# jessegrabowski/gEconpy

Measured on AMD Instinct MI355X. Metric: solve+Kalman-logp evals/sec, Smets-Wouters n~40 T=200, higher is better.
Workload: dtype f64; 1 GPU; sw_shaped synthetic (SURVEY 8d): n=m=40, n_state=18, n_lead=12, k=7, p=7, T_len=200, 4096 draws per GPU (BASELINE configs[2]); global_batch=4096, solver=cycle_reduction, inputs=A,B,C,D resident in HBM, parallelism=single GPU

## Files before the change

geconpy_amd/_lib.py:

```python
from __future__ import annotations

import ctypes as C
import os

PKG = os.path.dirname(os.path.abspath(__file__))
LIB_PATH = os.path.join(PKG, "libdsge_hip.so")

ABI_VERSION = 19
ERR_INVALID, ERR_HIP, ERR_TOO_LARGE = 1, 2, 3
MAX_N = 64
MAX_N_CR = 64
MAX_N_GENSYS = 64
MAX_N_BIG = 96
MAX_P = 16

ST_OK = 0
ST_NOT_CONVERGED = 1
ST_NAN = 2
ST_LYAP_FAIL = 4
ST_FILTER_NONFINITE = 8
ST_GENSYS_QZ_FAIL = 16
ST_GENSYS_TOO_BIG = 32
ST_GRAD_UNSUPPORTED = 64
ST_SECOND_ORDER_UNSUPPORTED = 128
# ... 39 lines not shown


class GensysForward(C.Structure):

    _fields_ = [("f_mat", C.c_void_p), ("f_wt", C.c_void_p), ("y_wt", C.c_void_p), ("loose", C.c_void_p),
                ("n_unstable", C.c_void_p), ("pi_raw", C.c_int32)]


_INTS = ("N T_len batch bound_batched c c_batched correlation cv_batched cv_paths d_batched device enable eps_batched "
         "eta_batched full_cov h_batched horizon k lag_step m max_iter mode n n_cond n_eta n_filter_hint n_grid n_groups n_lags "
         "n_lead n_lead_hint n_links n_out n_paths n_ret n_shock_steps n_state n_state_hint n_steps nnz p q_batched q_mode "
         "remainder reps s_batched shock solver w_batched x0_batched x0_paths z_batched z_selector_hint")
_KINDS = {**dict.fromkeys(_INTS.split(), C.c_int), **dict.fromkeys("jitter missing_fill rank_tol tol".split(), C.c_double),
          "scratch_limit_bytes": C.c_size_t}
_OBS = "Z z_batched d d_batched Hdiag h_batched"
_FILTER = f"T R Q q_mode {_OBS} y batch m k p T_len jitter missing_fill"
_FUSED = f"A B C D Q q_mode {_OBS} y batch n k p T_len solver tol max_iter jitter missing_fill"
_LOGP = f"{_FUSED} n_state_hint z_selector_hint n_lead_hint logp_out status_out"
_GRAD = f"A B C D q q_batched {_OBS} y batch n k p T_len solver tol max_iter jitter missing_fill"
_BARS = "logp_out status_out A_bar B_bar C_bar D_bar q_bar d_bar h_bar"
_PRUNED = "T R gyy gyu guu gss state_idx n_state"
_PENCIL = "g0 g1 *c psi pi batch N k n_eta tol G1_out C_out impact_out gev_out eu_out status"
_DEVICE_ENTRIES = {
    "dsge_abi_version": "",
    "dsge_last_error": "",
    "dsge_device_count": "",
    "dsge_set_device": "device",
    "dsge_stream_synchronize": "stream",
    "dsge_options_init": "opt",
    "dsge_options_push": "opt",
    "dsge_options_pop": "",
    "dsge_forget_measured_shapes": "",
    "dsge_debug_cr_phases": "enable cycles_out",
    "dsge_debug_kalman_steady_steps": "steady_at_device",
    "dsge_debug_kalman_timeline": "timeline_device",
    "dsge_debug_kalman_phases": "enable cycles_out",
    "dsge_debug_big_phases": "enable cycles_out",
    "dsge_debug_gensys_phases": "A B C batch n tol n_lead_hint T_out eu_out status cycles_out",
    "dsge_debug_gensys_window_phases": "enable cycles_out",
    "dsge_debug_gensys_stage_ms": "enable ms_out",
    "dsge_debug_adjoint_refine": "mode",
    "dsge_debug_second_order_phases": "enable cycles_out",
    "dsge_debug_pruned_phases": "enable cycles_out",
    "dsge_debug_shock_decomp_phases": "enable cycles_out",
    "dsge_debug_condfc_phases": "enable cycles_out",
    "dsge_profile_pipeline": f"{_LOGP} reps ms_out stream",
    "dsge_cycle_reduction_batched": "A B C batch n max_iter tol T_out status n_iter stream",
    "dsge_scan_cycle_reduction_batched": "A B C batch n max_iter tol T_out status *n_steps stream",
    "dsge_gensys_batched": "A B C D batch n k tol n_lead_hint T_out R_out eu_out status stream",
    "dsge_gensys_pencil_batched": f"{_PENCIL} stream",
    "dsge_gensys_pencil_full_batched": f"{_PENCIL} forward stream",
    "dsge_bk_eigenvalues_batched": "A B C batch n tol eig_re eig_im n_eig n_forward n_unstable status stream",
    "dsge_selection_batched": "A B C D T batch n k R_out resid_out stream",
    "dsge_policy_adjoints_batched": "B C T T_bar batch n A_bar B_bar C_bar status stream",
    "dsge_selection_adjoints_batched": "B C T R R_bar batch n k B_bar C_bar D_bar T_bar stream",
    "dsge_policy_norms_batched": "A B C D T R state_mask batch n k det_norm_out stoch_norm_out stream",
    "dsge_backward_direct_batched": "A B D batch n k T_out R_out stream",
    "dsge_lyapunov_batched": "T R Q q_mode batch m k P0_out RQR_out status stream",
    "dsge_autocorrelation_batched": "T R Q q_mode Z Hdiag batch m k p n_lags lag_step correlation acf_out Sigma_out status stream",
    "dsge_kalman_logp_batched": f"{_FILTER} n_state_hint z_selector_hint logp_out status_io stream",
    "dsge_kalman_filter_outputs_batched": f"{_FILTER} ll_out a_pred_out a_filt_out p_pred_out p_filt_out full_cov status_io stream",
    "dsge_kalman_smoother_batched": (f"{_FILTER} rank_tol scratch_limit_bytes ll_out a_smooth_out p_smooth_out eps_smooth_out "
                                     "full_cov status_io stream"),
    "dsge_simulation_smoother_batched": (f"{_FILTER} rank_tol scratch_limit_bytes x0 x0_batched eps eps_batched eta eta_batched "
                                         "n_paths ll_out x_out eps_out status_io stream"),
    "dsge_simulate_batched": "T R eps eps_batched x0 x0_batched status batch m k n_paths n_steps n_shock_steps x_out stream",
# ... 188 lines not shown
```

geconpy_amd/csrc/dsge_api.hip:

```cpp
#include <hip/hip_runtime.h>

#include <cmath>
#include <cstdio>
#include <cstdlib>
#include <cstring>
#include <mutex>
#include <string>
#include <vector>

#include "dsge_host.hpp"

namespace {
thread_local std::string g_last_error;
}

namespace dsge_host {
int fail(int code, const std::string& msg) {
  g_last_error = msg;
  return code;
}
static Options defaults_from_environment() {
  Options o;
  if (const char* e = std::getenv("DSGE_GENSYS_DOUBLING"))
    if ((e[0] >= '0' && e[0] <= '3') && e[1] == '\0') o.gensys_doubling = e[0] - '0';
// ... 224 lines not shown

namespace {
thread_local ThreadStream t_verdict;
constexpr int MAX_CHUNK_STREAMS = 8;
thread_local ThreadStream t_chunk[MAX_CHUNK_STREAMS];

StreamArenaPool g_scratch_pool;
StreamArenaPool g_aug_big_pool;
}

extern "C" {

int dsge_abi_version(void) { return DSGE_ABI_VERSION; }
const char* dsge_last_error(void) { return g_last_error.c_str(); }

static int debug_counters(long long** slot, int count, int enable, long long* cycles_out) {
  int rc = ensure_device();
  if (rc) return rc;
  if (enable && !*slot) {
    HIP_TRY(hipMalloc((void**)slot, count * sizeof(long long)));
    HIP_TRY(hipMemset(*slot, 0, count * sizeof(long long)));
  }
  if (cycles_out && *slot) {
    HIP_TRY(hipDeviceSynchronize());
    HIP_TRY(hipMemcpy(cycles_out, *slot, count * sizeof(long long), hipMemcpyDeviceToHost));
  }
  if (!enable && *slot) {
    (void)hipFree(*slot);
    *slot = nullptr;
  }
  return DSGE_SUCCESS;
}
int dsge_debug_cr_phases(int enable, long long* cycles_out) { return debug_counters(&g_cr_dbg, 8, enable, cycles_out); }
int dsge_debug_second_order_phases(int enable, long long* cycles_out) { return debug_counters(&g_so_dbg, 8, enable, cycles_out); }
int dsge_debug_pruned_phases(int enable, long long* cycles_out) { return debug_counters(&g_pruned_dbg, 8, enable, cycles_out); }
int dsge_debug_shock_decomp_phases(int enable, long long* cycles_out) { return debug_counters(&g_shock_decomp_dbg, 8, enable, cycles_out); }
int dsge_debug_condfc_phases(int enable, long long* cycles_out) { return debug_counters(&g_condfc_dbg, 8, enable, cycles_out); }
int dsge_debug_adjoint_refine(int mode) {
  if (mode < 0 || mode > 2) return fail(DSGE_ERR_INVALID, "mode out of range (0..2)");
  g_adj_refine_mode = mode;
  return DSGE_SUCCESS;
}
int dsge_forget_measured_shapes(void) {
  cr_deflation_reset();
  gensys_shape_reset();
  return DSGE_SUCCESS;
}
int dsge_debug_kalman_steady_steps(int32_t* steady_at_device) {
  g_kalman_steady_at = steady_at_device;
  return DSGE_SUCCESS;
}
int dsge_debug_kalman_timeline(long long* timeline_device) {
  g_kalman_timeline = timeline_device;
  return DSGE_SUCCESS;
}

int dsge_device_count(void) {
  int count = 0;
  if (hipGetDeviceCount(&count) != hipSuccess) {
    (void)hipGetLastError();
    return 0;
  }
  int ok = 0;
  for (int i = 0; i < count; ++i) {
    hipDeviceProp_t prop;
    if (hipGetDeviceProperties(&prop, i) == hipSuccess && std::strncmp(prop.gcnArchName, "gfx950", 6) == 0) ++ok;
// ... 1318 lines not shown
```

geconpy_amd/csrc/dsge_cr_compact.hpp:

```cpp
#pragma once
#include "dsge_device.hpp"

#include "../../include/dsge_hip.h"

namespace dsge {

template <int BS>
struct CrcSmem {
  static constexpr int NP = Tile<BS>::NP, LDW = 2 * NP + (BS % 2 == 0 ? 2 : 1);
  static constexpr size_t bytes = sizeof(double) * (size_t)(NP * LDW + NP * BS + BS * 2 * NP) + sizeof(int) * 5 * NP;
};

template <int BS>
__device__ __forceinline__ unsigned long long blk_colmask(const double (&x)[BS][BS]) {
  unsigned long long mask = 0ull;
#pragma unroll
  for (int j = 0; j < BS; ++j) {
    bool nz = false;
#pragma unroll
    for (int i = 0; i < BS; ++i) nz = nz || (x[i][j] != 0.0);
    unsigned long long b = __ballot(nz);
    b |= b >> 32;
    b |= b >> 16;
    b |= b >> 8;
    b &= 0xffull;
    while (b) {
      const int lcb = __ffsll((long long)b) - 1;
      b &= b - 1;
      const int col = lcb * BS + j;
      if (col < 64) mask |= 1ull << col;
    }
  }
  return mask;
}

template <int BS, typename IT>
__device__ __forceinline__ void crc_iterate(double (&A1)[BS][BS], double (&Ah)[BS][BS], double (&Rb)[BS][BS], double* W,
                                            double* Lbuf, double* Ybuf, int* prow, const IT* cmap, IT* rsrc,
                                            const IT* posS, const IT* posL, int n, int s, int l, int max_iter,
                                            double tol, int scan_mode, int lane_in, long long* ph, int& it, bool& converged,
                                            bool& saw_nan) {
  constexpr int NP = CrcSmem<BS>::NP, LDW = CrcSmem<BS>::LDW;
  double* G1 = W + NP;
// ... 65 lines not shown
    }
    wave_sync();
    if (ph) {
      const long long tk1 = clock64();
      ph[2] += tk1 - tk0;
      tk0 = tk1;
    }
    double acc1[BS][BS], acc2[BS][BS];
    blk_zero<BS>(acc1);
    blk_zero<BS>(acc2);
    mm_acc<BS, false>(acc1, G1, LDW, W, LDW, s, lr, lc);
    mm_acc<BS, false>(acc2, G1 + s, LDW, W + s * LDW, LDW, l, lr, lc);
    wave_sync();
    if (ph) {
      const long long tk1 = clock64();
      ph[3] += tk1 - tk0;
      tk0 = tk1;
    }
    blk_store_lds<BS>(acc1, W, LDW, lr, lc);
    blk_store_lds<BS>(acc2, G1, LDW, lr, lc);
    wave_sync();
    double t0[BS][BS], t2[BS][BS];
    int vS[BS], vL[BS];
#pragma unroll
    for (int j = 0; j < BS; ++j) {
      vS[j] = posS[lc * BS + j];
      vL[j] = posL[lc * BS + j];
    }
#pragma unroll
    for (int i = 0; i < BS; ++i)
#pragma unroll
      for (int j = 0; j < BS; ++j) {
        const int row = lr * BS + i, c = lc * BS + j;
        const double d02 = (vL[j] >= 0) ? W[row * LDW + vL[j]] : 0.0;
        const double d20 = (vS[j] >= 0) ? G1[row * LDW + vS[j]] : 0.0;
        A1[i][j] -= d02;
        A1[i][j] -= d20;
        Ah[i][j] -= d20;
        t0[i][j] = (c < s) ? acc1[i][j] : 0.0;
        t2[i][j] = (c >= s && c < wr) ? acc2[i][j] : 0.0;
        Rb[i][j] = -(t0[i][j] + t2[i][j]);
      }
    ++it;
    const double nrm0 = blk_norm1<BS>(t0);
    if (ph) ph[4] += clock64() - tk0;
    if (nrm0 < tol) {
      if (scan_mode || blk_norm1<BS>(t2) < tol) {
        converged = true;
        break;
      }
    } else if (nrm0 != nrm0) {
      saw_nan = true;
      break;
    }
    wave_sync();
  }
}

template <int BS>
__device__ __forceinline__ void cr_compact_body(const double* __restrict__ A, const double* __restrict__ B,
                                                const double* __restrict__ C, int batch, int n, int max_iter,
                                                double tol, double* __restrict__ T_out,
                                                int32_t* __restrict__ status,
                                                int32_t* __restrict__ n_iter_out,
                                                long long* __restrict__ dbg, int scan_mode,
                                                const double* __restrict__ D, int k,
                                                double* __restrict__ R_out) {
  constexpr int NP = CrcSmem<BS>::NP, LDW = CrcSmem<BS>::LDW;
// ... 1 lines not shown
  double* W = smem;
  double* G1 = W + NP;
  double* Lbuf = W + NP * LDW;
  double* Ybuf = Lbuf + NP * BS;
  int* prow = (int*)(Ybuf + BS * 2 * NP);
  int* cmap = prow + NP;
  int* posS = cmap + NP;
  int* posL = posS + NP;
  int* rsrc = posL + NP;
  const int lane = threadIdx.x, lr = lane >> 3, lc = lane & 7;

  for (int draw = blockIdx.x; draw < batch; draw = batch) {
    const size_t off = (size_t)draw * n * n;
    wave_sync();
    for (int idx = lane; idx < NP * LDW; idx += 64) W[idx] = 0.0;
    double A1[BS][BS], Ah[BS][BS], Rb[BS][BS];
    unsigned long long maskS, maskL;
    {
      double t[BS][BS];
      blk_load_global<BS>(t, A + off, n, n, n, lr, lc);
      maskS = blk_colmask<BS>(t);
      blk_load_global<BS>(t, C + off, n, n, n, lr, lc);
      maskL = blk_colmask<BS>(t);
    }
    const int s = __popcll(maskS), l = __popcll(maskL), wr = s + l;
    if (wr > NP) {
      if (lane == 0) status[draw] = DSGE_ST_INTERNAL_RERUN;
      continue;
    }
    if (lane < NP) {
      const unsigned long long below = (1ull << lane) - 1ull;
      const bool isS = (maskS >> lane) & 1ull, isL = (maskL >> lane) & 1ull;
      const int ps = __popcll(maskS & below), pl = s + __popcll(maskL & below);
      posS[lane] = isS ? ps : -1;
      posL[lane] = isL ? pl : -1;
      if (isS) cmap[ps] = lane;
      if (isL) cmap[pl] = lane;
    }
    wave_sync();
    int ccol[BS];
    int vS[BS], vL[BS];
#pragma unroll
    for (int j = 0; j < BS; ++j) {
      const int c = lc * BS + j;
      ccol[j] = (c < wr) ? cmap[c] : -1;
      vS[j] = posS[c];
      vL[j] = posL[c];
    }
#pragma unroll
    for (int i = 0; i < BS; ++i)
#pragma unroll
      for (int j = 0; j < BS; ++j) {
        const int r = lr * BS + i, c = lc * BS + j;
        double v = 0.0;
        if (r < n && ccol[j] >= 0) v = (c < s) ? A[off + (size_t)r * n + ccol[j]] : C[off + (size_t)r * n + ccol[j]];
        Rb[i][j] = v;
      }
    blk_load_global<BS>(A1, B + off, n, n, n, lr, lc);
#pragma unroll
    for (int i = 0; i < BS; ++i)
#pragma unroll
      for (int j = 0; j < BS; ++j) Ah[i][j] = A1[i][j];

    bool converged, saw_nan;
    int it;
    long long ph[8] = {0, 0, 0, 0, 0, 0, 0, 0};
    const long long tk_start = dbg ? clock64() : 0;
    crc_iterate<BS>(A1, Ah, Rb, W, Lbuf, Ybuf, prow, cmap, rsrc, posS, posL, n, s, l, max_iter, tol, scan_mode, lane,
// ... 2 lines not shown

    double Tb[BS][BS];
    blk_zero<BS>(Tb);
    const bool solve_T = converged || (scan_mode && !saw_nan);
    if (solve_T) {
      const bool want_R = (R_out != nullptr) && !scan_mode;
      const bool r_fits = want_R && (s + k <= NP);
      wave_sync();
      blk_store_lds<BS>(Ah, W, LDW, lr, lc);
      if (scan_mode && lr == lc) {
#pragma unroll
        for (int i = 0; i < BS; ++i) W[(lr * BS + i) * LDW + lc * BS + i] = Ah[i][i] + 1e-16;
      }
      {
        double t[BS][BS];
#pragma unroll
        for (int i = 0; i < BS; ++i)
#pragma unroll
          for (int j = 0; j < BS; ++j) {
            const int r = lr * BS + i, c = lc * BS + j;
            double v = 0.0;
            if (r < n && c < s) v = A[off + (size_t)r * n + ccol[j]];
            else if (r_fits && r < n && c >= s && c < s + k) v = D[(size_t)draw * n * k + (size_t)r * k + (c - s)];
            t[i][j] = v;
          }
        blk_store_lds<BS>(t, G1, LDW, lr, lc);
      }
      gauss_jordan_blocked<BS>(W, LDW, n, 2, Lbuf, Ybuf, prow, lane);
      gj_unpermute<BS>(W, LDW, n, 1, 2, prow, lane);
#pragma unroll
      for (int i = 0; i < BS; ++i)
#pragma unroll
        for (int j = 0; j < BS; ++j)
          Tb[i][j] = (vS[j] >= 0) ? -G1[(lr * BS + i) * LDW + vS[j]] : 0.0;
      if (r_fits) {
        for (int idx = lane; idx < n * k; idx += 64) {
          const int r = idx / k, c = idx - r * k;
          R_out[(size_t)draw * n * k + idx] = -G1[r * LDW + s + c];
        }
      } else if (want_R) {
        wave_sync();
        blk_store_lds<BS>(Ah, W, LDW, lr, lc);
        {
          double t[BS][BS];
          blk_load_global<BS>(t, D + (size_t)draw * n * k, n, k, k, lr, lc);
          blk_store_lds<BS>(t, G1, LDW, lr, lc);
        }
        gauss_jordan_blocked<BS>(W, LDW, n, 2, Lbuf, Ybuf, prow, lane);
        gj_unpermute<BS>(W, LDW, n, 1, 2, prow, lane);
        for (int idx = lane; idx < n * k; idx += 64) {
          const int r = idx / k, c = idx - r * k;
          R_out[(size_t)draw * n * k + idx] = -G1[r * LDW + c];
        }
      }
    }
    if (R_out != nullptr && !scan_mode && !solve_T)
      for (int idx = lane; idx < n * k; idx += 64) R_out[(size_t)draw * n * k + idx] = 0.0;
    blk_store_global<BS>(Tb, T_out + off, n, n, n, lr, lc);
    if (lane == 0) {
      status[draw] = solve_T ? DSGE_ST_OK : (DSGE_ST_NOT_CONVERGED | (saw_nan ? DSGE_ST_NAN : 0));
      if (n_iter_out) n_iter_out[draw] = it;
      if (dbg && draw == 0) {
        const long long tk_end = clock64();
        ph[5] = tk_end - tk_fin;
        ph[6] = tk_end - tk_start;
        ph[7] = it;
        for (int q = 0; q < 8; ++q) dbg[q] = ph[q];
// ... 27 lines not shown
```

geconpy_amd/csrc/dsge_cr_deflate.hpp:

```cpp
#pragma once
#include "dsge_device.hpp"

#include "../../include/dsge_hip.h"

namespace dsge {

constexpr int CRD_HMAX = 16;

__host__ __device__ inline size_t crd_top_doubles(int n, int k, int h) {
  return (size_t)h * (h + 3 * (n - h) + k) + 2;
}
__host__ __device__ inline size_t crd_deflate_smem(int tile) {
  return (size_t)(CRD_HMAX * tile + CRD_HMAX) * 8 + (64 + CRD_HMAX) * 4;
}
__host__ __device__ inline size_t crd_inflate_smem(int tile) {
  return (size_t)(2 * CRD_HMAX * tile + CRD_HMAX * CRD_HMAX + CRD_HMAX) * 8 + (64 + CRD_HMAX) * 4;
}

__global__ __launch_bounds__(64) void cr_static_scan_kernel(const double* __restrict__ A, const double* __restrict__ C,
                                                             int batch, int n, int32_t* __restrict__ out) {
  const int lane = threadIdx.x;
  for (int draw = blockIdx.x; draw < batch; draw += gridDim.x) {
    const size_t off = (size_t)draw * n * n;
    int nz = 0;
// ... 53 lines not shown
  }
  return keep;
}

template <typename IT>
__device__ __forceinline__ bool crd_col_source(int cv, const double* __restrict__ A, const double* __restrict__ B,
                                               const double* __restrict__ C, const double* __restrict__ D, size_t off,
                                               size_t offk, int n, int k, int h, const IT* dyi, const IT* sti,
                                               const double*& src, int& ss) {
  const int nd = n - h;
  src = B + off;
  ss = n;
  if (cv >= h + 3 * nd + k) return false;
  if (cv < h) {
    src = B + off + sti[cv];
    return true;
  }
  const int c = cv - h;
  if (c >= 3 * nd) {
    src = D + offk + (c - 3 * nd);
    ss = k;
    return true;
  }
  const int blk = (c >= nd) + (c >= 2 * nd);
  src = (blk == 0 ? B : (blk == 1 ? A : C)) + off + dyi[c - blk * nd];
  return true;
}

template <int NM, int NC, typename IT>
__device__ __forceinline__ void crd_qr_chunk(const double* __restrict__ A, const double* __restrict__ B,
                                             const double* __restrict__ C, const double* __restrict__ D, size_t off,
                                             size_t offk, int n, int k, int h, int c0, const IT* dyi, const IT* sti,
                                             double* V, double* __restrict__ tp, int lane, double (&col)[NC][NM],
                                             bool (&act)[NC], bool skip_zero_ac = false) {
  const int ncols = h + 3 * (n - h) + k;
  const double* src[NC];
  int ss[NC], cv[NC];
#pragma unroll
  for (int q = 0; q < NC; ++q) {
    cv[q] = c0 + 64 * q + lane;
    act[q] = crd_col_source(cv[q], A, B, C, D, off, offk, n, k, h, dyi, sti, src[q], ss[q]);
  }
#pragma unroll
  for (int r = 0; r < NM; ++r) {
    const int rr = r < n ? r : n - 1;
#pragma unroll
    for (int q = 0; q < NC; ++q) col[q][r] = src[q][(size_t)rr * ss[q]];
  }
  __builtin_amdgcn_sched_barrier(0);
#pragma unroll
  for (int r = 0; r < NM; ++r)
#pragma unroll
    for (int q = 0; q < NC; ++q) col[q][r] = (r < n && act[q]) ? col[q][r] : 0.0;
  bool wr[NC];
#pragma unroll
  for (int q = 0; q < NC; ++q) {
    wr[q] = act[q];
    if (skip_zero_ac) {
      bool nz = false;
#pragma unroll
      for (int r = 0; r < NM; ++r) nz = nz || (col[q][r] != 0.0);
      const int nd_ = n - h;
      const bool ac = cv[q] >= h + nd_ && cv[q] < h + 3 * nd_;
      wr[q] = act[q] && (nz || !ac);
    }
  }
  for (int j = 0; j < h; ++j) {
    double xn2 = 0.0, alpha;
    double d0[NC], d1[NC];
    if (c0 == 0) {
      if (lane == j) {
        double2* vw = reinterpret_cast<double2*>(V + j * NM);
#pragma unroll
        for (int r2 = 0; r2 < NM / 2; ++r2) vw[r2] = make_double2(col[0][2 * r2], col[0][2 * r2 + 1]);
      }
      wave_sync();
    }
    const double2* vj2 = reinterpret_cast<const double2*>(V + j * NM);
    {
      const double2 t0 = vj2[0];
      alpha = t0.x;
      xn2 = t0.y * t0.y;
#pragma unroll
      for (int q = 0; q < NC; ++q) {
        d0[q] = t0.y * col[q][1];
        d1[q] = 0.0;
      }
#pragma unroll
      for (int r2 = 1; r2 < NM / 2; ++r2) {
        const double2 t = vj2[r2];
        xn2 = fma(t.x, t.x, xn2);
#pragma unroll
        for (int q = 0; q < NC; ++q) d1[q] = fma(t.x, col[q][2 * r2], d1[q]);
        xn2 = fma(t.y, t.y, xn2);
#pragma unroll
        for (int q = 0; q < NC; ++q) d0[q] = fma(t.y, col[q][2 * r2 + 1], d0[q]);
      }
    }
    double beta = alpha, scal = 0.0, tj = 0.0;
    if (xn2 != 0.0) {
      const double nrm = sqrt(fma(alpha, alpha, xn2));
      beta = (alpha >= 0.0) ? -nrm : nrm;
      tj = (beta - alpha) / beta;
      scal = 1.0 / (alpha - beta);
    }
    const bool left = (c0 == 0) && (lane <= j);
    const double2 t0 = vj2[0];
#pragma unroll
    for (int q = 0; q < NC; ++q) {
      const bool lf = (q == 0) && left;
      const double w = lf ? 0.0 : -tj * fma(scal, d0[q] + d1[q], col[q][0]);
      const double topv = lf ? ((lane == j) ? beta : 0.0) : col[q][0] + w;
      if (wr[q]) tp[(size_t)j * ncols + cv[q]] = topv;
      const double ws = w * scal;
      col[q][0] = lf ? 0.0 : fma(t0.y, ws, col[q][1]);
#pragma unroll
      for (int r2 = 1; r2 < NM / 2; ++r2) {
        const double2 t = vj2[r2];
        col[q][2 * r2 - 1] = lf ? 0.0 : fma(t.x, ws, col[q][2 * r2]);
        col[q][2 * r2] = lf ? 0.0 : fma(t.y, ws, col[q][2 * r2 + 1]);
      }
      col[q][NM - 1] = 0.0;
    }
  }
}

template <int BS>
__global__ __launch_bounds__(64) void cr_deflate_kernel(const double* __restrict__ A, const double* __restrict__ B,
                                                         const double* __restrict__ C, const double* __restrict__ D,
                                                         int batch, int n, int k, int h, double* __restrict__ Ared,
                                                         double* __restrict__ Bred, double* __restrict__ Cred,
                                                         double* __restrict__ Dred, double* __restrict__ top,
                                                         int32_t* __restrict__ flag) {
  constexpr int NM = 8 * BS, HM = CRD_HMAX;
  extern __shared__ __attribute__((aligned(16))) double smem[];
  double* V = smem;
  double* tau_s = V + HM * NM;
  int* dyi = (int*)(tau_s + HM);
  int* sti = dyi + 64;
  const int lane = threadIdx.x;
  const int nd = n - h, nv = 3 * nd + k, ncols = h + nv;
  const size_t top_stride = crd_top_doubles(n, k, h);
  {
    const int draw = blockIdx.x;
    if (draw >= batch) return;
    const size_t off = (size_t)draw * n * n, offk = (size_t)draw * n * k;
    const size_t offr = (size_t)draw * nd * nd, offrk = (size_t)draw * nd * k;
    unsigned long long smask = crd_static_mask<NM>(A, C, off, n, lane);
    if (__popcll(smask) < h) {
      for (int idx = lane; idx < nd * nd; idx += 64) {
        Ared[offr + idx] = 0.0;
        Cred[offr + idx] = 0.0;
        Bred[offr + idx] = (idx / nd == idx % nd) ? 1.0 : 0.0;
// ... 240 lines not shown
```

geconpy_amd/csrc/dsge_cr_fused.hpp:

```cpp
#pragma once
#include "dsge_cr_compact.hpp"
#include "dsge_cr_deflate.hpp"

namespace dsge {

template <int BSF, int BSD>
struct CrfSmem {
  static constexpr int NMF = 8 * BSF, NPD = 8 * BSD, LDW = CrcSmem<BSD>::LDW, HM = CRD_HMAX;
  static constexpr size_t dbl_compact = (size_t)(NPD * LDW + NPD * BSD + BSD * 2 * NPD);
  static constexpr size_t dbl_qr = (size_t)(HM * NMF + HM);
  static constexpr size_t dbl_inflate = CrdInflateLds<NPD>::doubles;
  static constexpr size_t dbl =
      dbl_compact > dbl_qr ? (dbl_compact > dbl_inflate ? dbl_compact : dbl_inflate) : (dbl_qr > dbl_inflate ? dbl_qr : dbl_inflate);
  typedef signed char idx_t;
  static constexpr size_t bytes = sizeof(double) * dbl + sizeof(int) * NPD + ((4 * NPD + 64 + HM + 15) & ~(size_t)15);
};

__host__ __device__ inline size_t crf_rhs_doubles(int nd, int npd) { return (size_t)nd * npd; }

__device__ __forceinline__ unsigned long long crf_place(unsigned long long b, int shift) {
  return shift >= 0 ? (shift < 64 ? b << shift : 0ull) : (-shift < 64 ? b >> (-shift) : 0ull);
}

template <int BSF, int BSD, int NC>
__device__ __forceinline__ void cr_fused_body(const double* __restrict__ A, const double* __restrict__ B,
                                              const double* __restrict__ C, const double* __restrict__ D, int batch, int n,
                                              int k, int h, int max_iter, double tol, double* __restrict__ top,
                                              double* __restrict__ rhs, double* __restrict__ T_out,
                                              double* __restrict__ R_out, int32_t* __restrict__ status,
                                              int32_t* __restrict__ n_iter_out,
                                              unsigned long long* __restrict__ colmask_out) {
  using SM = CrfSmem<BSF, BSD>;
  constexpr int NMF = SM::NMF, NPD = SM::NPD, LDW = SM::LDW, HM = CRD_HMAX;
  extern __shared__ __attribute__((aligned(16))) double smem[];
  double* W = smem;
  double* G1 = W + NPD;
  double* Lbuf = W + NPD * LDW;
  double* Ybuf = Lbuf + NPD * BSD;
  typedef typename SM::idx_t idx_t;
  int* prow = (int*)(smem + SM::dbl);
  idx_t* cmap = (idx_t*)(prow + NPD);
  idx_t* posS = cmap + NPD;
  idx_t* posL = posS + NPD;
  idx_t* rsrc = posL + NPD;
  idx_t* dyi = rsrc + NPD;
  idx_t* sti = dyi + 64;
  const int lane = threadIdx.x, lr = lane >> 3, lc = lane & 7;
  const int nd = n - h;
  const int draw = blockIdx.x;
  if (draw >= batch) return;
  const size_t off = (size_t)draw * n * n, offk = (size_t)draw * n * k;
  auto hand_over = [&]() {
    if (lane == 0) {
      status[draw] = DSGE_ST_INTERNAL_RERUN;
      if (colmask_out) colmask_out[draw] = ~0ull;
    }
  };
  if (colmask_out && lane == 0) colmask_out[draw] = ~0ull;

  unsigned long long smask = crd_static_mask<NMF>(A, C, off, n, lane);
  if (__popcll(smask) < h) return hand_over();
  smask = crd_first_bits(smask, h);
  crd_index_tables(smask, n, lane, dyi, sti);
  double* tp = top + (size_t)draw * crd_top_doubles(n, k, h);
  double* rh = rhs + (size_t)draw * crf_rhs_doubles(nd, NPD);
  int s, l;
  unsigned long long state_cols = 0ull, maskS_red = 0ull, maskL_red = 0ull;
  {
    double col[NC][NMF];
    bool act[NC];
    crd_qr_chunk<NMF, NC>(A, B, C, D, off, offk, n, k, h, 0, dyi, sti, smem, tp, lane, col, act,
                          true);
    int blk[NC], dcol[NC];
    unsigned long long bS = 0ull, bL = 0ull;
#pragma unroll
    for (int q = 0; q < NC; ++q) {
      const int c = 64 * q + lane - h;
      blk[q] = -1;
      dcol[q] = 0;
      if (act[q] && c >= 0) {
        blk[q] = (c >= nd) + (c >= 2 * nd) + (c >= 3 * nd);
        dcol[q] = c - blk[q] * nd;
      }
      bool nz = false;
#pragma unroll
      for (int r = 0; r < NMF; ++r) nz = nz || (col[q][r] != 0.0);
      bS |= crf_place(__ballot(blk[q] == 1 && nz), 64 * q - (h + nd));
      bL |= crf_place(__ballot(blk[q] == 2 && nz), 64 * q - (h + 2 * nd));
    }
    const unsigned long long ndmask = (nd >= 64) ? ~0ull : ((1ull << nd) - 1ull);
    const unsigned long long maskS = bS & ndmask, maskL = bL & ndmask;
    s = __popcll(maskS);
    l = __popcll(maskL);
    maskS_red = maskS;
    maskL_red = maskL;
    if (s + l > NPD || s + k > NPD) return hand_over();
    {
      const unsigned long long below = (1ull << lane) - 1ull;
      const bool dyn = (lane < n) && !((smask >> lane) & 1ull);
      const int dred = lane - __popcll(smask & below);
      state_cols = __ballot(dyn && ((maskS >> (dred & 63)) & 1ull));
    }
    wave_sync();
    for (int idx = lane; idx < NPD * LDW; idx += 64) W[idx] = 0.0;
    if (lane < NPD) {
      const unsigned long long below = (1ull << lane) - 1ull;
      const bool isS = (maskS >> lane) & 1ull, isL = (maskL >> lane) & 1ull;
      const int ps = __popcll(maskS & below), pl = s + __popcll(maskL & below);
      posS[lane] = (idx_t)(isS ? ps : -1);
      posL[lane] = (idx_t)(isL ? pl : -1);
      if (isS) cmap[ps] = (idx_t)lane;
      if (isL) cmap[pl] = (idx_t)lane;
    }
    wave_sync();
#pragma unroll
    for (int q = 0; q < NC; ++q) {
      const int d = dcol[q];
      const unsigned long long below = (1ull << d) - 1ull;
      int lcol = -1, gcol = -1;
      if (blk[q] == 0) {
        lcol = d;
      } else if (blk[q] == 1) {
        if ((maskS >> d) & 1ull) {
          gcol = __popcll(maskS & below);
          lcol = NPD + gcol;
        }
      } else if (blk[q] == 2) {
        if ((maskL >> d) & 1ull) lcol = NPD + s + __popcll(maskL & below);
      } else if (blk[q] == 3) {
        gcol = s + d;
      }
      if (lcol >= 0) {
        double* dst = W + lcol;
#pragma unroll
        for (int r = 0; r < NMF; ++r)
          if (r < nd) dst[r * LDW] = col[q][r];
      }
      if (gcol >= 0) {
        double* dst = rh + (size_t)gcol * nd;
#pragma unroll
        for (int r = 0; r < NMF; ++r)
          if (r < nd) dst[r] = col[q][r];
      }
    }
  }
  wave_sync();

  double A1[BSD][BSD], Ah[BSD][BSD], Rb[BSD][BSD];
  blk_load_lds<BSD>(A1, W, LDW, lr, lc);
  blk_load_lds<BSD>(Rb, G1, LDW, lr, lc);
  int vS[BSD], vL[BSD];
#pragma unroll
  for (int j = 0; j < BSD; ++j) {
    vS[j] = posS[lc * BSD + j];
    vL[j] = posL[lc * BSD + j];
  }
#pragma unroll
  for (int i = 0; i < BSD; ++i)
#pragma unroll
    for (int j = 0; j < BSD; ++j) Ah[i][j] = A1[i][j];
  wave_sync();
  bool converged, saw_nan;
  int it;
  crc_iterate<BSD>(A1, Ah, Rb, W, Lbuf, Ybuf, prow, cmap, rsrc, posS, posL, nd, s, l, max_iter, tol, 0, lane, nullptr, it,
                   converged, saw_nan);
  if (lane == 0) {
    status[draw] = converged ? DSGE_ST_OK : (DSGE_ST_NOT_CONVERGED | (saw_nan ? DSGE_ST_NAN : 0));
    if (n_iter_out) n_iter_out[draw] = it;
  }
  if (!converged) {
    for (int idx = lane; idx < n * n; idx += 64) T_out[off + idx] = 0.0;
    for (int idx = lane; idx < n * k; idx += 64) R_out[offk + idx] = 0.0;
    return;
  }
  wave_sync();
  int lane_f = lane;
  asm volatile("" : "+v"(lane_f));
  {
    int lane_s = lane;
    asm volatile("" : "+v"(lane_s));
    const int lr_s = lane_s >> 3, lc_s = lane_s & 7;
    blk_store_lds<BSD>(Ah, W, LDW, lr_s, lc_s);
    double t[BSD][BSD];
#pragma unroll
    for (int i = 0; i < BSD; ++i)
#pragma unroll
      for (int j = 0; j < BSD; ++j) {
        const int r = lr_s * BSD + i, c = lc_s * BSD + j;
        t[i][j] = (r < nd && c < s + k) ? rh[(size_t)c * nd + r] : 0.0;
      }
    blk_store_lds<BSD>(t, G1, LDW, lr_s, lc_s);
  }
  gauss_jordan_blocked<BSD>(W, LDW, nd, 2, Lbuf, Ybuf, prow, lane_f);
  gj_unpermute<BSD>(W, LDW, nd, 1, 2, prow, lane_f);

  double y[NPD];
  {
    const int ntot = nd + k;
    int src = -1;
    if (lane < nd)
      src = posS[lane];
    else if (lane < ntot)
      src = s + (lane - nd);
#pragma unroll
    for (int q = 0; q < NPD; ++q) y[q] = (q < nd && src >= 0) ? -G1[q * LDW + src] : 0.0;
  }
  wave_sync();
  const CrdInflateLds<NPD> L(smem);
  if (!crd_inflate_prepare<NPD>(y, lane < nd + k, tp, n, k, h, lane, L, maskL_red)) return hand_over();
  if (lane < n) {
#pragma unroll
    for (int s2 = 0; s2 < HM; ++s2)
      if (s2 < h) T_out[off + (size_t)lane * n + sti[s2]] = 0.0;
  }
  crd_inflate_chunk<NPD>(0, y, tp, n, k, h, lane, L, dyi, sti, T_out + off, R_out + offk, maskS_red);
  if (colmask_out && lane == 0) colmask_out[draw] = state_cols;
}

template <int BSF, int BSD, int NC = 2>
__global__ __launch_bounds__(64) void cr_fused_kernel(const double* __restrict__ A, const double* __restrict__ B,
                                                       const double* __restrict__ C, const double* __restrict__ D, int batch,
                                                       int n, int k, int h, int max_iter, double tol,
                                                       double* __restrict__ top, double* __restrict__ rhs,
                                                       double* __restrict__ T_out, double* __restrict__ R_out,
                                                       int32_t* __restrict__ status, int32_t* __restrict__ n_iter_out,
                                                       unsigned long long* __restrict__ colmask_out) {
  cr_fused_body<BSF, BSD, NC>(A, B, C, D, batch, n, k, h, max_iter, tol, top, rhs, T_out, R_out, status, n_iter_out, colmask_out);
}

template <int BSF, int BSD>
__global__ __launch_bounds__(64) __attribute__((amdgpu_waves_per_eu(2, 2))) void cr_fused_kernel_occ2(
    const double* __restrict__ A, const double* __restrict__ B, const double* __restrict__ C, const double* __restrict__ D,
    int batch, int n, int k, int h, int max_iter, double tol, double* __restrict__ top, double* __restrict__ rhs,
    double* __restrict__ T_out, double* __restrict__ R_out, int32_t* __restrict__ status, int32_t* __restrict__ n_iter_out,
    unsigned long long* __restrict__ colmask_out) {
  cr_fused_body<BSF, BSD, 2>(A, B, C, D, batch, n, k, h, max_iter, tol, top, rhs, T_out, R_out, status, n_iter_out, colmask_out);
}

}
```

geconpy_amd/csrc/dsge_host.hpp:

```cpp
#pragma once
#include <hip/hip_runtime.h>
#include <stdint.h>

#include <mutex>
#include <string>
#include <vector>

#include "../../include/dsge_hip.h"
#include "dsge_filter_conv.hpp"

namespace dsge_host {

int fail(int code, const std::string& msg);

#define HIP_TRY(expr)                                                                              \
  do {                                                                                             \
    hipError_t _e = (expr);                                                                        \
    if (_e != hipSuccess) {                                                                        \
      (void)hipGetLastError();         \
      return dsge_host::fail(DSGE_ERR_HIP, std::string(#expr) + ": " + hipGetErrorString(_e));     \
    }                                                                                              \
  } while (0)

constexpr size_t LDS_LIMIT = 160 * 1024;
// ... 325 lines not shown
  int used = 0;
};
int launch_gensys_overlap_merge(int batch, const int32_t* marks, const int32_t* vstatus, int32_t* status, double* logp,
                                hipStream_t st);
int launch_gensys(const double* A, const double* B, const double* C, int batch, int n, double tol, int n_lead_hint,
                  double* T_out, int32_t* eu_out, int32_t* status, hipStream_t st, long long* dbg = nullptr,
                  int32_t* key_out = nullptr, int* key_written = nullptr,
                  const double* D = nullptr, int k = 0, double* R_tmp = nullptr, int n_state_hint = 0,
                  const int32_t** qz_marks = nullptr,
                  GensysOverlap* ov = nullptr);

int launch_gensys_pencil(const double* g0, const double* g1, const double* c, const double* psi, const double* pi, int batch,
                         int N, int k, int ell, double tol, double* G1_out, double* C_out, double* impact_out,
                         double* gev_out, int32_t* eu_out, int32_t* status, hipStream_t st,
                         const dsge_gensys_forward* fw = nullptr);

int launch_gensys_bk(const double* A, const double* B, const double* C, int batch, int n, double tol, double* eig_re,
                     double* eig_im, int32_t* n_eig, int32_t* n_forward, int32_t* n_unstable, int32_t* status,
                     hipStream_t st);

int launch_second_order(const double* B, const double* C, const double* T, const double* R, const int32_t* hess_idx, int nnz,
                        const double* hess_val, const double* q, int q_batched, const double* Z, const double* d,
                        const double* Hdiag, const double* y, int batch, int n, int k, int p, int T_len, double jitter,
                        double missing_fill, const int32_t* S, int s, const int32_t* L, int l, const int32_t* U, int u,
                        double* logp, int32_t* status_io, double* gyy_out, double* gyu_out, double* guu_out, double* gss_out,
                        int32_t* steady_at, int32_t* n_doublings, hipStream_t st, float* ms, const int32_t* order_key = nullptr);

extern int g_adj_refine_mode;
extern long long* g_so_dbg;
extern long long* g_pruned_dbg;
extern long long* g_shock_decomp_dbg;
extern long long* g_condfc_dbg;
extern long long* g_cr_dbg;
extern long long* g_big_dbg;
extern long long* g_kalman_dbg;
extern long long* g_gensys_win_dbg;
extern float* g_gensys_stage_ms;
extern long long* g_kalman_timeline;
extern int32_t* g_kalman_steady_at;

struct Options : dsge_options {
  int grad_fused_adjoint = 1;
  Options() : dsge_options{} {
    struct_size = (uint32_t)sizeof(dsge_options);
    cr_compact = 1;
    cr_fused_selection = 1;
    cr_deflation = 1;
    cr_two_waves = 1;
    n_static_hint = -1;
    kalman_order = 1;
    kalman_tiny = 1;
    kalman_block = 0;
    kalman_mfma = 2;
    cr_four_waves = 1;
    cr_fused_deflation = 1;
    kalman_nt_products = 1;
    pipeline_chunks = 0;
    gensys_split = 1;
    gensys_real_stage = 1;
    kalman_steady_tol = 1e-14;
    gensys_pairs = 1;
    gensys_shape_cache = 1;
    gensys_direct_blocks = 1;
    kalman_narrow = 1;
    gensys_doubling = 1;
    kalman_grad_split = 2;
// ... 302 lines not shown
```

geconpy_amd/csrc/launch_solvers.hip:

```cpp
#include "dsge_host.hpp"
#include "dsge_kernels.hpp"
#include "dsge_cr_compact.hpp"
#include "dsge_cr_deflate.hpp"
#include "dsge_cr_fused.hpp"
#include "dsge_cr_wide.hpp"

#include <algorithm>
#include <mutex>

namespace dsge_host {

long long* g_cr_dbg = nullptr;


int launch_cr(const double* A, const double* B, const double* C, int batch, int n, int max_iter, double tol,
              double* T_out, int32_t* status, int32_t* n_iter, hipStream_t st, int scan_mode, const double* D, int k,
              double* R_out) {
  const int bs = tile_bs(n);
  int rc = DSGE_ERR_INVALID;
  const bool compact = opt().cr_compact != 0;
  if (compact && n > 48 && opt().cr_four_waves) {
    if ((rc = set_lds(dsge::cr_wide_kernel, dsge::CrwSmem::bytes))) return rc;
    hipLaunchKernelGGL(dsge::cr_wide_kernel, dim3(batch), dim3(256), dsge::CrwSmem::bytes, st, A, B, C, batch, n, max_iter, tol,
                       T_out, status, n_iter, scan_mode, D, k, R_out);
    HIP_TRY(hipGetLastError());
  } else if (compact) {
    DISPATCH_BS(bs, 8, {
      if (BS == 4 && opt().cr_two_waves) {
        rc = set_lds(dsge::cr_compact_kernel_occ2<4>, dsge::CrcSmem<4>::bytes);
        if (rc == DSGE_SUCCESS) {
          hipLaunchKernelGGL(dsge::cr_compact_kernel_occ2<4>, dim3(batch), dim3(64), dsge::CrcSmem<4>::bytes, st, A, B, C,
                             batch, n, max_iter, tol, T_out, status, n_iter, g_cr_dbg, scan_mode, D, k, R_out);
          HIP_TRY(hipGetLastError());
        }
      } else {
        rc = set_lds(dsge::cr_compact_kernel<BS>, dsge::CrcSmem<BS>::bytes);
        if (rc == DSGE_SUCCESS) {
          hipLaunchKernelGGL(dsge::cr_compact_kernel<BS>, dim3(batch), dim3(64), dsge::CrcSmem<BS>::bytes, st, A, B, C,
                             batch, n, max_iter, tol, T_out, status, n_iter, g_cr_dbg, scan_mode, D, k, R_out);
          HIP_TRY(hipGetLastError());
        }
      }
    });
    if (rc) return rc;
  }
  rc = DSGE_ERR_INVALID;
// ... 1 lines not shown
    rc = set_lds(dsge::cr_kernel<BS>, dsge::CrSmem<BS>::bytes);
    if (rc == DSGE_SUCCESS) {
      hipLaunchKernelGGL(dsge::cr_kernel<BS>, dim3(compact ? rerun_grid(batch) : batch), dim3(64), dsge::CrSmem<BS>::bytes, st, A,
                         B, C, batch, n, max_iter, tol, T_out, status, n_iter, compact ? 1 : 0, scan_mode, D, k, R_out);
      HIP_TRY(hipGetLastError());
    }
  });
  return rc;
}


namespace {
std::mutex g_defl_mutex;
int g_static_hint[DSGE_MAX_N + 2];
unsigned g_static_calls[DSGE_MAX_N + 2];
bool g_static_hint_init = false;
StreamArenaPool g_defl_pool;
}

void cr_deflation_reset() {
  std::lock_guard<std::mutex> lk(g_defl_mutex);
  g_static_hint_init = false;
}

namespace {
template <int BSF, int BSD, int NC>
int launch_cr_fused_inst(const double* A, const double* B, const double* C, const double* D, int batch, int n, int k, int h,
                         int max_iter, double tol, double* top, double* rhs, double* T_out, double* R_out, int32_t* status,
                         int32_t* n_iter, hipStream_t st, unsigned long long* colmask) {
  using SM = dsge::CrfSmem<BSF, BSD>;
  int rc;
  if constexpr (BSD == 4 && NC == 2) {
    if (opt().cr_two_waves) {
      if ((rc = set_lds(dsge::cr_fused_kernel_occ2<BSF, BSD>, SM::bytes))) return rc;
      hipLaunchKernelGGL((dsge::cr_fused_kernel_occ2<BSF, BSD>), dim3(batch), dim3(64), SM::bytes, st, A, B, C, D, batch, n, k, h,
                         max_iter, tol, top, rhs, T_out, R_out, status, n_iter, colmask);
      HIP_TRY(hipGetLastError());
      return DSGE_SUCCESS;
    }
  }
  if ((rc = set_lds(dsge::cr_fused_kernel<BSF, BSD, NC>, SM::bytes))) return rc;
  hipLaunchKernelGGL((dsge::cr_fused_kernel<BSF, BSD, NC>), dim3(batch), dim3(64), SM::bytes, st, A, B, C, D, batch, n, k, h,
                     max_iter, tol, top, rhs, T_out, R_out, status, n_iter, colmask);
  HIP_TRY(hipGetLastError());
  return DSGE_SUCCESS;
}
}

int launch_cr_fused(const double* A, const double* B, const double* C, const double* D, int batch, int n, int k, int h,
                    int max_iter, double tol, double* T_out, double* R_out, int32_t* status, int32_t* n_iter, hipStream_t st,
                    int* done, unsigned long long* colmask) {
  *done = 0;
  const int nd = n - h, bsf = tile_bs(n), bsd = tile_bs(nd);
  const int ncol = h + 3 * nd + k, nc = ncol <= 128 ? 2 : 3;
  if (ncol > 192 || nd + k > 64) return DSGE_SUCCESS;
  const bool have = nc == 2 ? ((bsf == 3 && (bsd == 2 || bsd == 3)) || (bsf == 4 && (bsd == 3 || bsd == 4)) ||
                               (bsf == 5 && bsd == 4) || (bsf == 6 && (bsd == 4 || bsd == 5)))
                            : ((bsf == 6 && bsd == 5) || (bsf == 7 && (bsd == 5 || bsd == 6)) || (bsf == 8 && bsd == 6));
  if (!have) return DSGE_SUCCESS;
  int rc;
  double *top = nullptr, *rhs = nullptr;
  ScratchLayout lay;
  lay.add(&top, (size_t)batch * dsge::crd_top_doubles(n, k, h));
  lay.add(&rhs, (size_t)batch * dsge::crf_rhs_doubles(nd, 8 * bsd));
  if ((rc = lay.reserve(g_defl_pool, st))) return rc;
#define FUSED_CASE(F, D_, N_)                                                                                          \
// ... 138 lines not shown
```

include/dsge_hip.h:

```cpp
#ifndef DSGE_HIP_H
#define DSGE_HIP_H

#include <stddef.h>
#include <stdint.h>

#ifdef __cplusplus
extern "C" {
#endif

#define DSGE_ABI_VERSION 19


#define DSGE_MAX_N 64
#define DSGE_MAX_N_CR 64
#define DSGE_MAX_N_GENSYS 64
#define DSGE_MAX_N_BIG 96
#define DSGE_MAX_P 16
#define DSGE_SPECTRAL_MAX_K 32
#define DSGE_SPECTRAL_MAX_P 64
#define DSGE_SPECTRAL_MAX_GRID 4096
#define DSGE_ANT_MAX_LEAD 63
#define DSGE_OBC_MAX_HORIZON 64

#define DSGE_SUCCESS 0
// ... 67 lines not shown
  int32_t kalman_order;
  int32_t kalman_tiny;
  int32_t kalman_block;
  int32_t kalman_mfma;
  int32_t pipeline_chunks;
  int32_t gensys_split;
  double kalman_steady_tol;
  int32_t kalman_nt_products;
  int32_t cr_fused_deflation;
  int32_t cr_four_waves;
  int32_t gensys_real_stage;
  int32_t gensys_pairs;
  int32_t gensys_shape_cache;
  int32_t kalman_narrow;
  int32_t gensys_direct_blocks;
  int32_t ll_constant;
  int32_t mask_d;
  int32_t joseph;
  int32_t kalman_head_draws;
  double jitter_F;
  double jitter_P;
  int32_t gensys_doubling;
  int32_t kalman_grad_split;
  int32_t reserved_[2];
} dsge_options;
int dsge_options_init(dsge_options* opt);
int dsge_options_push(const dsge_options* opt);
int dsge_options_pop(void);
int dsge_forget_measured_shapes(void);


int dsge_debug_cr_phases(int enable, long long* cycles_out);

int dsge_gensys_batched(const double* A, const double* B, const double* C, const double* D, int batch, int n,
                        int k, double tol, int n_lead_hint, double* T_out, double* R_out, int32_t* eu_out,
                        int32_t* status, void* stream);
int dsge_gensys_batched_host(const double* A, const double* B, const double* C, const double* D, int batch,
                             int n, int k, double tol, int n_lead_hint, double* T_out, double* R_out,
                             int32_t* eu_out, int32_t* status);

int dsge_gensys_pencil_batched(const double* g0, const double* g1, const double* c, const double* psi, const double* pi,
                               int batch, int N, int k, int n_eta, double tol, double* G1_out, double* C_out,
                               double* impact_out, double* gev_out, int32_t* eu_out, int32_t* status, void* stream);
int dsge_gensys_pencil_batched_host(const double* g0, const double* g1, const double* c, const double* psi,
                                    const double* pi, int batch, int N, int k, int n_eta, double tol, double* G1_out,
                                    double* C_out, double* impact_out, double* gev_out, int32_t* eu_out,
                                    int32_t* status);

typedef struct dsge_gensys_forward {
  double* f_mat;
  double* f_wt;
  double* y_wt;
  double* loose;
  int32_t* n_unstable;
  int32_t pi_raw;
} dsge_gensys_forward;
int dsge_gensys_pencil_full_batched(const double* g0, const double* g1, const double* c, const double* psi,
                                    const double* pi, int batch, int N, int k, int n_eta, double tol, double* G1_out,
                                    double* C_out, double* impact_out, double* gev_out, int32_t* eu_out,
                                    int32_t* status, const dsge_gensys_forward* forward, void* stream);
int dsge_gensys_pencil_full_batched_host(const double* g0, const double* g1, const double* c, const double* psi,
                                         const double* pi, int batch, int N, int k, int n_eta, double tol,
                                         double* G1_out, double* C_out, double* impact_out, double* gev_out,
                                         int32_t* eu_out, int32_t* status, const dsge_gensys_forward* forward);

int dsge_bk_eigenvalues_batched(const double* A, const double* B, const double* C, int batch, int n, double tol,
// ... 372 lines not shown
```

Before: 3.356 million evals/s.

## Pad CR column positions, fold final solve into RHS elimination, add fused-CR phase probe

```diff
diff --git a/geconpy_amd/_lib.py b/geconpy_amd/_lib.py
--- a/geconpy_amd/_lib.py
+++ b/geconpy_amd/_lib.py
@@ -95,6 +95,7 @@
     "dsge_options_pop": "",
     "dsge_forget_measured_shapes": "",
     "dsge_debug_cr_phases": "enable cycles_out",
+    "dsge_debug_cr_fused_phases": "enable cycles_out",
     "dsge_debug_kalman_steady_steps": "steady_at_device",
     "dsge_debug_kalman_timeline": "timeline_device",
     "dsge_debug_kalman_phases": "enable cycles_out",
diff --git a/geconpy_amd/csrc/dsge_api.hip b/geconpy_amd/csrc/dsge_api.hip
--- a/geconpy_amd/csrc/dsge_api.hip
+++ b/geconpy_amd/csrc/dsge_api.hip
@@ -280,6 +280,7 @@
   return DSGE_SUCCESS;
 }
 int dsge_debug_cr_phases(int enable, long long* cycles_out) { return debug_counters(&g_cr_dbg, 8, enable, cycles_out); }
+int dsge_debug_cr_fused_phases(int enable, long long* cycles_out) { return debug_counters(&g_cr_fused_dbg, 16, enable, cycles_out); }
 int dsge_debug_second_order_phases(int enable, long long* cycles_out) { return debug_counters(&g_so_dbg, 8, enable, cycles_out); }
 int dsge_debug_pruned_phases(int enable, long long* cycles_out) { return debug_counters(&g_pruned_dbg, 8, enable, cycles_out); }
 int dsge_debug_shock_decomp_phases(int enable, long long* cycles_out) { return debug_counters(&g_shock_decomp_dbg, 8, enable, cycles_out); }
diff --git a/geconpy_amd/csrc/dsge_cr_compact.hpp b/geconpy_amd/csrc/dsge_cr_compact.hpp
--- a/geconpy_amd/csrc/dsge_cr_compact.hpp
+++ b/geconpy_amd/csrc/dsge_cr_compact.hpp
@@ -2,6 +2,8 @@
 #include "dsge_device.hpp"
 
 #include "../../include/dsge_hip.h"
+
+#include <limits>
 
 namespace dsge {
 
@@ -9,6 +11,13 @@
 struct CrcSmem {
   static constexpr int NP = Tile<BS>::NP, LDW = 2 * NP + (BS % 2 == 0 ? 2 : 1);
   static constexpr size_t bytes = sizeof(double) * (size_t)(NP * LDW + NP * BS + BS * 2 * NP) + sizeof(int) * 5 * NP;
+};
+
+template <int BS, typename IT>
+struct CrcPos {
+  static constexpr int NP = 8 * BS;
+  static constexpr bool pad = 2 * NP <= (int)std::numeric_limits<IT>::max();
+  static constexpr int noS = pad ? NP : -1, noL = pad ? 2 * NP : -1;
 };
 
 template <int BS>
@@ -140,8 +149,14 @@
 #pragma unroll
       for (int j = 0; j < BS; ++j) {
         const int row = lr * BS + i, c = lc * BS + j;
-        const double d02 = (vL[j] >= 0) ? W[row * LDW + vL[j]] : 0.0;
-        const double d20 = (vS[j] >= 0) ? G1[row * LDW + vS[j]] : 0.0;
+        double d02, d20;
+        if constexpr (CrcPos<BS, IT>::pad) {
+          d02 = W[row * LDW + vL[j]];
+          d20 = G1[row * LDW + vS[j]];
+        } else {
+          d02 = (vL[j] >= 0) ? W[row * LDW + vL[j]] : 0.0;
+          d20 = (vS[j] >= 0) ? G1[row * LDW + vS[j]] : 0.0;
+        }
         A1[i][j] -= d02;
         A1[i][j] -= d20;
         Ah[i][j] -= d20;
@@ -209,8 +224,8 @@
       const unsigned long long below = (1ull << lane) - 1ull;
       const bool isS = (maskS >> lane) & 1ull, isL = (maskL >> lane) & 1ull;
       const int ps = __popcll(maskS & below), pl = s + __popcll(maskL & below);
-      posS[lane] = isS ? ps : -1;
-      posL[lane] = isL ? pl : -1;
+      posS[lane] = isS ? ps : CrcPos<BS, int>::noS;
+      posL[lane] = isL ? pl : CrcPos<BS, int>::noL;
       if (isS) cmap[ps] = lane;
       if (isL) cmap[pl] = lane;
     }
@@ -279,7 +294,7 @@
       for (int i = 0; i < BS; ++i)
 #pragma unroll
         for (int j = 0; j < BS; ++j)
-          Tb[i][j] = (vS[j] >= 0) ? -G1[(lr * BS + i) * LDW + vS[j]] : 0.0;
+          Tb[i][j] = (vS[j] != CrcPos<BS, int>::noS) ? -G1[(lr * BS + i) * LDW + vS[j]] : 0.0;
       if (r_fits) {
         for (int idx = lane; idx < n * k; idx += 64) {
           const int r = idx / k, c = idx - r * k;
diff --git a/geconpy_amd/csrc/dsge_cr_deflate.hpp b/geconpy_amd/csrc/dsge_cr_deflate.hpp
--- a/geconpy_amd/csrc/dsge_cr_deflate.hpp
+++ b/geconpy_amd/csrc/dsge_cr_deflate.hpp
@@ -109,7 +109,8 @@
                                              const double* __restrict__ C, const double* __restrict__ D, size_t off,
                                              size_t offk, int n, int k, int h, int c0, const IT* dyi, const IT* sti,
                                              double* V, double* __restrict__ tp, int lane, double (&col)[NC][NM],
-                                             bool (&act)[NC], bool skip_zero_ac = false) {
+                                             bool (&act)[NC], bool skip_zero_ac = false,
+                                             long long* t_loaded = nullptr) {
   const int ncols = h + 3 * (n - h) + k;
   const double* src[NC];
   int ss[NC], cv[NC];
@@ -142,6 +143,7 @@
       wr[q] = act[q] && (nz || !ac);
     }
   }
+  if (t_loaded) *t_loaded = clock64();
   for (int j = 0; j < h; ++j) {
     double xn2 = 0.0, alpha;
     double d0[NC], d1[NC];
@@ -190,12 +192,12 @@
       const double topv = lf ? ((lane == j) ? beta : 0.0) : col[q][0] + w;
       if (wr[q]) tp[(size_t)j * ncols + cv[q]] = topv;
       const double ws = w * scal;
-      col[q][0] = lf ? 0.0 : fma(t0.y, ws, col[q][1]);
+      col[q][0] = fma(t0.y, ws, col[q][1]);
 #pragma unroll
       for (int r2 = 1; r2 < NM / 2; ++r2) {
         const double2 t = vj2[r2];
-        col[q][2 * r2 - 1] = lf ? 0.0 : fma(t.x, ws, col[q][2 * r2]);
-        col[q][2 * r2] = lf ? 0.0 : fma(t.y, ws, col[q][2 * r2 + 1]);
+        col[q][2 * r2 - 1] = fma(t.x, ws, col[q][2 * r2]);
+        col[q][2 * r2] = fma(t.y, ws, col[q][2 * r2 + 1]);
       }
       col[q][NM - 1] = 0.0;
     }
diff --git a/geconpy_amd/csrc/dsge_cr_fused.hpp b/geconpy_amd/csrc/dsge_cr_fused.hpp
--- a/geconpy_amd/csrc/dsge_cr_fused.hpp
+++ b/geconpy_amd/csrc/dsge_cr_fused.hpp
@@ -22,14 +22,15 @@
   return shift >= 0 ? (shift < 64 ? b << shift : 0ull) : (-shift < 64 ? b >> (-shift) : 0ull);
 }
 
-template <int BSF, int BSD, int NC>
+template <int BSF, int BSD, int NC, bool DBG = false>
 __device__ __forceinline__ void cr_fused_body(const double* __restrict__ A, const double* __restrict__ B,
                                               const double* __restrict__ C, const double* __restrict__ D, int batch, int n,
                                               int k, int h, int max_iter, double tol, double* __restrict__ top,
                                               double* __restrict__ rhs, double* __restrict__ T_out,
                                               double* __restrict__ R_out, int32_t* __restrict__ status,
                                               int32_t* __restrict__ n_iter_out,
-                                              unsigned long long* __restrict__ colmask_out) {
+                                              unsigned long long* __restrict__ colmask_out,
+                                              long long* __restrict__ dbg = nullptr) {
   using SM = CrfSmem<BSF, BSD>;
   constexpr int NMF = SM::NMF, NPD = SM::NPD, LDW = SM::LDW, HM = CRD_HMAX;
   extern __shared__ __attribute__((aligned(16))) double smem[];
@@ -58,6 +59,8 @@
   };
   if (colmask_out && lane == 0) colmask_out[draw] = ~0ull;
 
+  long long tk_start = 0, tk_ld = 0, tk_qr = 0;
+  if constexpr (DBG) tk_start = clock64();
   unsigned long long smask = crd_static_mask<NMF>(A, C, off, n, lane);
   if (__popcll(smask) < h) return hand_over();
   smask = crd_first_bits(smask, h);
@@ -70,7 +73,8 @@
     double col[NC][NMF];
     bool act[NC];
     crd_qr_chunk<NMF, NC>(A, B, C, D, off, offk, n, k, h, 0, dyi, sti, smem, tp, lane, col, act,
-                          true);
+                          true, DBG ? &tk_ld : nullptr);
+    if constexpr (DBG) tk_qr = clock64();
     int blk[NC], dcol[NC];
     unsigned long long bS = 0ull, bL = 0ull;
 #pragma unroll
@@ -107,8 +111,8 @@
       const unsigned long long below = (1ull << lane) - 1ull;
       const bool isS = (maskS >> lane) & 1ull, isL = (maskL >> lane) & 1ull;
       const int ps = __popcll(maskS & below), pl = s + __popcll(maskL & below);
-      posS[lane] = (idx_t)(isS ? ps : -1);
-      posL[lane] = (idx_t)(isL ? pl : -1);
+      posS[lane] = (idx_t)(isS ? ps : CrcPos<BSD, idx_t>::noS);
+      posL[lane] = (idx_t)(isL ? pl : CrcPos<BSD, idx_t>::noL);
       if (isS) cmap[ps] = (idx_t)lane;
       if (isL) cmap[pl] = (idx_t)lane;
     }
@@ -162,8 +166,12 @@
   wave_sync();
   bool converged, saw_nan;
   int it;
-  crc_iterate<BSD>(A1, Ah, Rb, W, Lbuf, Ybuf, prow, cmap, rsrc, posS, posL, nd, s, l, max_iter, tol, 0, lane, nullptr, it,
-                   converged, saw_nan);
+  long long ph[8] = {0, 0, 0, 0, 0, 0, 0, 0};
+  long long tk_dep = 0, tk_it = 0, tk_fin = 0;
+  if constexpr (DBG) tk_dep = clock64();
+  crc_iterate<BSD>(A1, Ah, Rb, W, Lbuf, Ybuf, prow, cmap, rsrc, posS, posL, nd, s, l, max_iter, tol, 0, lane,
+                   DBG ? ph : nullptr, it, converged, saw_nan);
+  if constexpr (DBG) tk_it = clock64();
   if (lane == 0) {
     status[draw] = converged ? DSGE_ST_OK : (DSGE_ST_NOT_CONVERGED | (saw_nan ? DSGE_ST_NAN : 0));
     if (n_iter_out) n_iter_out[draw] = it;
@@ -189,21 +197,23 @@
         const int r = lr_s * BSD + i, c = lc_s * BSD + j;
         t[i][j] = (r < nd && c < s + k) ? rh[(size_t)c * nd + r] : 0.0;
       }
+    double inv_lo = 1e300, inv_hi = 0.0;
+    gauss_jordan_blocked_rhs<BSD>(W, LDW, nd, t, Lbuf, Ybuf, prow, lane_f, nullptr, inv_lo, inv_hi);
     blk_store_lds<BSD>(t, G1, LDW, lr_s, lc_s);
   }
-  gauss_jordan_blocked<BSD>(W, LDW, nd, 2, Lbuf, Ybuf, prow, lane_f);
-  gj_unpermute<BSD>(W, LDW, nd, 1, 2, prow, lane_f);
-
+  wave_sync();
+
+  if constexpr (DBG) tk_fin = clock64();
   double y[NPD];
   {
     const int ntot = nd + k;
     int src = -1;
     if (lane < nd)
-      src = posS[lane];
+      src = (posS[lane] != CrcPos<BSD, idx_t>::noS) ? posS[lane] : -1;
     else if (lane < ntot)
       src = s + (lane - nd);
 #pragma unroll
-    for (int q = 0; q < NPD; ++q) y[q] = (q < nd && src >= 0) ? -G1[q * LDW + src] : 0.0;
+    for (int q = 0; q < NPD; ++q) y[q] = (q < nd && src >= 0) ? -G1[prow[q < nd ? q : 0] * LDW + src] : 0.0;
   }
   wave_sync();
   const CrdInflateLds<NPD> L(smem);
@@ -215,6 +225,19 @@
   }
   crd_inflate_chunk<NPD>(0, y, tp, n, k, h, lane, L, dyi, sti, T_out + off, R_out + offk, maskS_red);
   if (colmask_out && lane == 0) colmask_out[draw] = state_cols;
+  if constexpr (DBG) {
+    if (dbg && draw == 0 && lane == 0) {
+      const long long tk_end = clock64();
+      for (int q = 0; q < 5; ++q) dbg[q] = ph[q];
+      dbg[5] = tk_fin - tk_it;
+      dbg[6] = tk_end - tk_start;
+      dbg[7] = it;
+      dbg[8] = tk_ld - tk_start;
+      dbg[9] = tk_qr - tk_ld;
+      dbg[10] = tk_dep - tk_qr;
+      dbg[11] = tk_end - tk_fin;
+    }
+  }
 }
 
 template <int BSF, int BSD, int NC = 2>
@@ -237,4 +260,14 @@
   cr_fused_body<BSF, BSD, 2>(A, B, C, D, batch, n, k, h, max_iter, tol, top, rhs, T_out, R_out, status, n_iter_out, colmask_out);
 }
 
-}
+template <int BSF, int BSD>
+__global__ __launch_bounds__(64) __attribute__((amdgpu_waves_per_eu(2, 2))) void cr_fused_kernel_occ2_dbg(
+    const double* __restrict__ A, const double* __restrict__ B, const double* __restrict__ C, const double* __restrict__ D,
+    int batch, int n, int k, int h, int max_iter, double tol, double* __restrict__ top, double* __restrict__ rhs,
+    double* __restrict__ T_out, double* __restrict__ R_out, int32_t* __restrict__ status, int32_t* __restrict__ n_iter_out,
+    unsigned long long* __restrict__ colmask_out, long long* __restrict__ dbg) {
+  cr_fused_body<BSF, BSD, 2, true>(A, B, C, D, batch, n, k, h, max_iter, tol, top, rhs, T_out, R_out, status, n_iter_out,
+                                   colmask_out, dbg);
+}
+
+}
diff --git a/geconpy_amd/csrc/dsge_host.hpp b/geconpy_amd/csrc/dsge_host.hpp
--- a/geconpy_amd/csrc/dsge_host.hpp
+++ b/geconpy_amd/csrc/dsge_host.hpp
@@ -381,6 +381,7 @@
 extern long long* g_shock_decomp_dbg;
 extern long long* g_condfc_dbg;
 extern long long* g_cr_dbg;
+extern long long* g_cr_fused_dbg;
 extern long long* g_big_dbg;
 extern long long* g_kalman_dbg;
 extern long long* g_gensys_win_dbg;
diff --git a/geconpy_amd/csrc/launch_solvers.hip b/geconpy_amd/csrc/launch_solvers.hip
--- a/geconpy_amd/csrc/launch_solvers.hip
+++ b/geconpy_amd/csrc/launch_solvers.hip
@@ -11,7 +11,7 @@
 namespace dsge_host {
 
 long long* g_cr_dbg = nullptr;
-
+long long* g_cr_fused_dbg = nullptr;
 
 int launch_cr(const double* A, const double* B, const double* C, int batch, int n, int max_iter, double tol,
               double* T_out, int32_t* status, int32_t* n_iter, hipStream_t st, int scan_mode, const double* D, int k,
@@ -79,6 +79,15 @@
   int rc;
   if constexpr (BSD == 4 && NC == 2) {
     if (opt().cr_two_waves) {
+      if constexpr (BSF == 5) {
+        if (g_cr_fused_dbg) {
+          if ((rc = set_lds(dsge::cr_fused_kernel_occ2_dbg<BSF, BSD>, SM::bytes))) return rc;
+          hipLaunchKernelGGL((dsge::cr_fused_kernel_occ2_dbg<BSF, BSD>), dim3(batch), dim3(64), SM::bytes, st, A, B, C, D, batch, n,
+                             k, h, max_iter, tol, top, rhs, T_out, R_out, status, n_iter, colmask, g_cr_fused_dbg);
+          HIP_TRY(hipGetLastError());
+          return DSGE_SUCCESS;
+        }
+      }
       if ((rc = set_lds(dsge::cr_fused_kernel_occ2<BSF, BSD>, SM::bytes))) return rc;
       hipLaunchKernelGGL((dsge::cr_fused_kernel_occ2<BSF, BSD>), dim3(batch), dim3(64), SM::bytes, st, A, B, C, D, batch, n, k, h,
                          max_iter, tol, top, rhs, T_out, R_out, status, n_iter, colmask);
diff --git a/include/dsge_hip.h b/include/dsge_hip.h
--- a/include/dsge_hip.h
+++ b/include/dsge_hip.h
@@ -123,6 +123,8 @@
 
 int dsge_debug_cr_phases(int enable, long long* cycles_out);
 
+int dsge_debug_cr_fused_phases(int enable, long long* cycles_out);
+
 int dsge_gensys_batched(const double* A, const double* B, const double* C, const double* D, int batch, int n,
                         int k, double tol, int n_lead_hint, double* T_out, double* R_out, int32_t* eu_out,
                         int32_t* status, void* stream);
```

Result: faster. 3.407 million evals/s (median of 6 runs) (+1.5%).
